# ronantakizawa/cudabulletproof

Measured on AMD Instinct MI355X. Metric: 64-bit range-proof verifies/sec (batched), higher is better.
Workload: dtype u64

## Files before the change

### cudabulletproof_amd/csrc/bp_ipa_prove.hip

```cpp
#include "bp_kernels.h"
#include "ge25519_dev.h"
#include "sha256_dev.h"

namespace bp {

namespace {
constexpr int TPB = 256;
__device__ __forceinline__ size_t gid() { return (size_t)blockIdx.x * blockDim.x + threadIdx.x; }
inline unsigned nblk(size_t items) { return (unsigned)((items + TPB - 1) / TPB); }

__device__ __forceinline__ int sclass(const fe& s) {
    if (s.v[3] | s.v[2] | s.v[1]) return 2;
    return s.v[0] ? 1 : 0;
}

constexpr int CTL_HEAVY = MSM_BINS, CTL_LIGHT = MSM_BINS + 1;

__device__ __forceinline__ void block_hist(const IpaWs& ws, unsigned* hb, bool heavy, int key) {
    for (int k = threadIdx.x; k <= MSM_BINS; k += TPB) hb[k] = 0;
    __syncthreads();
    if (heavy) {
        atomicAdd(&hb[key], 1u);
        atomicAdd(&hb[MSM_BINS], 1u);
    }
    __syncthreads();
    for (int k = threadIdx.x; k <= MSM_BINS; k += TPB)
        if (hb[k]) atomicAdd(&ws.ctl[k], hb[k]);
}
}

__global__ __launch_bounds__(TPB) void k_ipa_elem(IpaWs ws, int np) {
    __shared__ unsigned hb[MSM_BINS + 1];
    const size_t i = gid(), per = 4 * (size_t)np;
    const bool live = i < (size_t)ws.B * per;
    bool heavy = false;
    int key = 0;
    if (live) {
        const size_t p = i / per;
        const int k = (int)(i % per), blk = k / np, j = k % np;
        const size_t n = (size_t)ws.n;
        const fe* a = ws.a + p * n;
        const fe* b = ws.b + p * n;
        const int hi = (blk == 1 || blk == 2) ? np : 0;
        const fe src = (blk & 1) ? b[hi + j] : a[hi + j];
        const fe s = fe_canon(src);
        ws.sc[p * 2 * n + k] = s;
        if (!(blk & 1))
            ws.prod[p * n + hi + j] = fe_mul(src, b[(np - hi) + j]);
        heavy = sclass(s) == 2;
        if (heavy) key = sm_ops_prefix(s, ws.ptab ? ws.pbits : 0);
    }
    block_hist(ws, hb, heavy, key);
}

__global__ __launch_bounds__(TPB) void k_ipa_cchain(IpaWs ws, int np) {
    __shared__ unsigned hb[MSM_BINS + 1];
    const size_t c = gid();
    const bool live = c < (size_t)ws.B * 2;
    bool heavy = false;
    int key = 0;
    if (live) {
        const fe* pr = ws.prod + (c >> 1) * (size_t)ws.n + (c & 1) * (size_t)np;
        fe acc = fe_set(0);
        for (int j = 0; j < np; j++) acc = fe_add(acc, pr[j]);
        const fe s = fe_canon(acc);
        ws.csc[c] = s;
        heavy = sclass(s) == 2;
        if (heavy) key = sm_ops_prefix(s, ws.ptab ? ws.pbits : 0);
    }
    block_hist(ws, hb, heavy, key);
}

__device__ __forceinline__ fe item_scalar(const IpaWs& ws, size_t p, int k, int np) {
    return k < 4 * np ? ws.sc[p * 2 * (size_t)ws.n + k] : ws.csc[p * 2 + (k - 4 * np)];
}
__device__ __forceinline__ ge* item_term(const IpaWs& ws, size_t p, int k, int np) {
    return k < 4 * np ? ws.term + p * 2 * (size_t)ws.n + k : ws.cq + p * 2 + (k - 4 * np);
}

__global__ __launch_bounds__(TPB) void k_ipa_scatter(IpaWs ws, int np, const ge* __restrict__ dtab) {
    __shared__ unsigned cnt[MSM_BINS + 1], base[MSM_BINS + 1];
    for (int k = threadIdx.x; k <= MSM_BINS; k += TPB) cnt[k] = 0;
    __syncthreads();
    const size_t i = gid(), per = 4 * (size_t)np + 2;
    int key = -1;
    unsigned rank = 0;
    if (i < (size_t)ws.B * per) {
        const size_t p = i / per;
        const int k = (int)(i % per);
        const fe s = item_scalar(ws, p, k, np);
        const int c = sclass(s);
        if (c == 0) *item_term(ws, p, k, np) = dtab[k < 4 * np ? 257 : 256];
        else key = c == 2 ? sm_ops_prefix(s, ws.ptab ? ws.pbits : 0) : MSM_BINS;
        if (key >= 0) rank = atomicAdd(&cnt[key], 1u);
    }
    __syncthreads();
    for (int k = threadIdx.x; k <= MSM_BINS; k += TPB)
        if (cnt[k]) base[k] = atomicAdd(&ws.ctl[k < MSM_BINS ? k : CTL_LIGHT], cnt[k]);
    __syncthreads();
    if (key >= 0) (key < MSM_BINS ? ws.slist : ws.llist)[base[key] + rank] = (uint32_t)i;
}

__global__ __launch_bounds__(TPB, 3) void k_ipa_terms(IpaWs ws, int np, const ge* __restrict__ G,
                                                   const ge* __restrict__ H, const ge* __restrict__ Q,
                                                   const ge* __restrict__ dtab) {
    __shared__ geq qs[TPB];
    const int n = ws.n;
    const size_t per = 4 * (size_t)np + 2;
    const unsigned ch = ws.ctl[CTL_HEAVY], cl = ws.ctl[CTL_LIGHT];
    for (size_t i = gid(); i < (size_t)ch + cl; i += (size_t)gridDim.x * TPB) {
        const uint32_t id = i < ch ? ws.slist[i] : ws.llist[i - ch];
        const size_t p = id / per;
        const int k = (int)(id % per);
        const bool msm = k < 4 * np;
        ge P;
        int base;
        if (msm) {
            const int blk = k / np, j = k % np;
            P = blk == 0 ? G[np + j] : blk == 1 ? H[j] : blk == 2 ? G[j] : H[np + j];
            base = blk == 0 ? np + j : blk == 1 ? n + j : blk == 2 ? j : n + np + j;
        } else {
            P = *Q;
            base = 2 * n;
        }
        const fe s = item_scalar(ws, p, k, np);
        const ge* pt = ws.ptab ? ws.ptab + ((size_t)base << ws.pbits) : nullptr;
        ge r = scalarmult<true>(s, P, &qs[threadIdx.x], dtab, pt, pt ? ws.pbits : 0);
        *item_term(ws, p, k, np) = msm ? ge_norm_host(r) : r;
    }
}

__global__ __launch_bounds__(TPB) void k_ipa_pchain(IpaWs ws, int np) {
    const size_t c = gid();
    if (c >= (size_t)ws.B * 4) return;
    const ge* t = ws.term + (c >> 2) * 2 * (size_t)ws.n + (c & 3) * (size_t)np;
    ge acc = t[0];
    for (int i = 1; i < np; i++) acc = ge_norm_host(ge_add(acc, t[i]));
    ws.chain[c] = ge_norm_host(acc);
}

__global__ __launch_bounds__(TPB) void k_ipa_round(IpaWs ws, int r) {
    const size_t p = gid();
    if (p >= (size_t)ws.B) return;
    const ge* ch = ws.chain + p * 4;
    const ge* tq = ws.cq + p * 2;
    const ge L = ge_norm_host(ge_add(ge_add(ge_add(ge_zero(), ch[0]), ch[1]), tq[0]));
    const ge R = ge_norm_host(ge_add(ge_add(ge_add(ge_zero(), ch[2]), ch[3]), tq[1]));
    ws.L[p * ws.Lr + r] = L;
    ws.R[p * ws.Lr + r] = R;
    const fe u = chal_ip(ws.tr[p], L.X, R.X);
    ws.tr[p] = u;
    if (r == 0) ws.x[p] = u;
    ws.uu[p * 2] = u;
    ws.uu[p * 2 + 1] = fe_invert(u);
}

__global__ __launch_bounds__(TPB) void k_ipa_fold(IpaWs ws, int np) {
    const size_t i = gid();
    if (i >= (size_t)ws.B * np) return;
    const size_t p = i / np;
    const int j = (int)(i % np);
    const fe u = ws.uu[p * 2], ui = ws.uu[p * 2 + 1];
    fe* a = ws.a + p * (size_t)ws.n;
    fe* b = ws.b + p * (size_t)ws.n;
    const fe na = fe_add(fe_mul(ui, a[j]), fe_mul(u, a[np + j]));
    const fe nb = fe_add(fe_mul(u, b[j]), fe_mul(ui, b[np + j]));
    a[j] = na;
    b[j] = nb;
}

__global__ __launch_bounds__(TPB) void k_ipa_load(IpaWs ws, const fe* __restrict__ a, const fe* __restrict__ b,
                                                  const fe* __restrict__ tr) {
    const size_t i = gid(), m = (size_t)ws.B * ws.n;
    if (i < m) {
        ws.a[i] = a[i];
        ws.b[i] = b[i];
    }
    if (i < (size_t)ws.B) {
        ws.tr[i] = tr ? tr[i] : fe_set(0);
        ws.x[i] = fe_set(0);
    }
}

__global__ __launch_bounds__(TPB) void k_ipa_final(IpaWs ws, const fe* __restrict__ c_in, fe* a, fe* b, fe* c,
                                                   fe* x, fe* c_final) {
    const size_t p = gid();
    if (p >= (size_t)ws.B) return;
    const fe fa = ws.a[p * (size_t)ws.n], fb = ws.b[p * (size_t)ws.n];
    a[p] = fa;
// ... 33 lines not shown
```

### cudabulletproof_amd/csrc/bp_kernels.hip

```cpp
#include "bp_kernels.h"
#include "ge25519_dev.h"
#include "ge25519_quad.h"
#include "sha256_dev.h"

namespace bp {

constexpr int TPB = 256;
#ifndef BP_TERMS_OCC
#define BP_TERMS_OCC 4
#endif


__device__ __forceinline__ size_t gid() { return (size_t)blockIdx.x * blockDim.x + threadIdx.x; }

__global__ __launch_bounds__(TPB) void k_prefix_tables(ge* tab, const ge* __restrict__ G, const ge* __restrict__ H,
                                                       const ge* __restrict__ h, const ge* __restrict__ g, int n,
                                                       int K, size_t total) {
    const size_t i = gid();
    if (i >= total) return;
    const size_t b = i >> K;
    const uint32_t p = (uint32_t)(i & ((1ull << K) - 1));
    const ge* P = b < (size_t)n ? &G[b] : b < 2 * (size_t)n ? &H[b - n] : b == 2 * (size_t)n ? h : g;
    if (!P) return;
    const geq q = ge_prep(*P);
    ge r = ge_zero();
    for (int j = K - 1; j >= 0; j--) {
        r = ge_add_sel<false>(r, &q, false);
        if ((p >> j) & 1) r = ge_add_sel<false>(r, &q, true);
    }
    tab[i] = r;
}

void launch_prefix_tables(ge* tab, const ge* G, const ge* H, const ge* h, const ge* g, int n, int K, hipStream_t s) {
    const size_t total = (size_t)(2 * n + 2) << K;
    k_prefix_tables<<<(unsigned)((total + TPB - 1) / TPB), TPB, 0, s>>>(tab, G, H, h, g, n, K, total);
}

#ifndef BP_MSM_TPB
#define BP_MSM_TPB 256
#endif
constexpr int MSM_TPB = BP_MSM_TPB;
__global__ __launch_bounds__(MSM_TPB, 768 / MSM_TPB) void k_msm_points(ge* pts, const fe* __restrict__ scal,
                                                    const ge* __restrict__ P, size_t total, size_t pm,
                                                    const uint32_t* __restrict__ perm,
                                                    const ge* __restrict__ dtab, const ge* __restrict__ ptab,
                                                    int K) {
    __shared__ geq qs[MSM_TPB];
    size_t i = gid();
    if (i >= total) return;
    if (perm) i = perm[i];
    const size_t b = pm == total ? i : i % pm;
    ge r = scalarmult<true>(scal[i], P[b], &qs[threadIdx.x], dtab, ptab ? ptab + (b << K) : nullptr, ptab ? K : 0);
    pts[i] = ge_norm_dev(r);
}

constexpr int OPS_BINS = MSM_BINS;

__global__ void k_ops_zero(unsigned* bins) {
    for (int k = threadIdx.x; k < OPS_BINS; k += blockDim.x) bins[k] = 0;
}

__global__ __launch_bounds__(TPB) void k_ops_hist(unsigned* bins, const fe* __restrict__ scal, size_t n, int K) {
    __shared__ unsigned h[OPS_BINS];
    for (int k = threadIdx.x; k < OPS_BINS; k += TPB) h[k] = 0;
    __syncthreads();
    size_t i = gid();
    if (i < n) atomicAdd(&h[sm_ops_prefix(scal[i], K)], 1u);
    __syncthreads();
    for (int k = threadIdx.x; k < OPS_BINS; k += TPB)
        if (h[k]) atomicAdd(&bins[k], h[k]);
}

constexpr int SCAN_T = 1024;
static_assert(OPS_BINS <= SCAN_T, "one scan block");
__global__ __launch_bounds__(SCAN_T) void k_ops_scan(unsigned* bins, int longest_first) {
    __shared__ unsigned a[SCAN_T];
    const int t = threadIdx.x;
    const int k = longest_first ? OPS_BINS - 1 - t : t;
    const unsigned v = t < OPS_BINS ? bins[k] : 0u;
    a[t] = v;
    __syncthreads();
    for (int off = 1; off < SCAN_T; off <<= 1) {
        unsigned x = t >= off ? a[t - off] : 0u;
        __syncthreads();
        a[t] += x;
        __syncthreads();
    }
    if (t < OPS_BINS) bins[k] = a[t] - v;
}

__global__ __launch_bounds__(SCAN_T) void k_ops_scatter(uint32_t* perm, unsigned* offs, const fe* __restrict__ scal,
                                                        size_t n, int K) {
    __shared__ unsigned cnt[OPS_BINS], base[OPS_BINS];
    for (int k = threadIdx.x; k < OPS_BINS; k += SCAN_T) cnt[k] = 0;
    __syncthreads();
    size_t i = (size_t)blockIdx.x * SCAN_T + threadIdx.x;
    int key = 0;
    unsigned rank = 0;
    if (i < n) {
        key = sm_ops_prefix(scal[i], K);
        rank = atomicAdd(&cnt[key], 1u);
    }
    __syncthreads();
    for (int k = threadIdx.x; k < OPS_BINS; k += SCAN_T)
        if (cnt[k]) base[k] = atomicAdd(&offs[k], cnt[k]);
    __syncthreads();
    if (i < n) perm[base[key] + rank] = (uint32_t)i;
}

void launch_ops_scan(unsigned* bins, int longest_first, hipStream_t s) {
    k_ops_scan<<<1, SCAN_T, 0, s>>>(bins, longest_first);
}

void launch_msm_points(ge* pts, const fe* scal, const ge* P, size_t m, uint32_t* perm, unsigned* bins,
                       const ge* dtab, hipStream_t s, size_t pm, const ge* ptab, int K) {
    if (!ptab) K = 0;
    if (!pm) pm = m;
    size_t blocks = (m + TPB - 1) / TPB;
    static const int sort_mode = getenv("HIPBP_MSM_SORT") ? atoi(getenv("HIPBP_MSM_SORT")) : 1;
    if (!sort_mode) perm = nullptr;
    if (perm && bins && m >= MSM_SORT_MIN && m <= 0xFFFFFFFFull) {
        k_ops_zero<<<1, 64, 0, s>>>(bins);
        k_ops_hist<<<blocks, TPB, 0, s>>>(bins, scal, m, K);
        k_ops_scan<<<1, SCAN_T, 0, s>>>(bins, sort_mode == 1);
        k_ops_scatter<<<(unsigned)((m + SCAN_T - 1) / SCAN_T), SCAN_T, 0, s>>>(perm, bins, scal, m, K);
    } else {
        perm = nullptr;
    }
    k_msm_points<<<(unsigned)((m + MSM_TPB - 1) / MSM_TPB), MSM_TPB, 0, s>>>(pts, scal, P, m, pm, perm, dtab, ptab, K);
}

__global__ __launch_bounds__(TPB) void k_tree(ge* out, const ge* __restrict__ in, size_t m, int nb) {
    __shared__ ge sh[TPB];
    int seg = blockIdx.x / nb, chunk = blockIdx.x % nb;
    int tid = threadIdx.x;
// ... 382 lines not shown
```

### cudabulletproof_amd/csrc/bp_prove.hip

```cpp
#include "bp_kernels.h"
#include "ge25519_dev.h"
#include "sha256_dev.h"

#ifndef BP_GTAB
#define BP_GTAB 1
#endif

namespace bp {

namespace {
constexpr int TPB = 256;
__device__ __forceinline__ size_t gid() { return (size_t)blockIdx.x * blockDim.x + threadIdx.x; }
inline unsigned nblk(size_t items) { return (unsigned)((items + TPB - 1) / TPB); }
}

__device__ __forceinline__ const ge* prow(const ProveWs& ws, int b) {
    return ws.ptab ? ws.ptab + ((size_t)b << ws.pbits) : nullptr;
}

__device__ __forceinline__ ge sm_norm(const fe& s, const ge& P, geq* qslot, const ge* __restrict__ dtab,
                                      const ge* pt, int K) {
    return ge_norm_host(scalarmult<true>(s, P, qslot, dtab, pt, pt ? K : 0));
}

// ... 36 lines not shown
}

__device__ __forceinline__ bool next_item(const ProveWs& ws, size_t i, uint32_t& id) {
    const unsigned ch = ws.cnt[0], cl = ws.cnt[1];
    if (i < ch) { id = ws.list[i]; return true; }
    if (i < (size_t)ch + cl) { id = ws.list[ws.cap + (i - ch)]; return true; }
    return false;
}

__device__ __forceinline__ fe terms0_scalar(const ProveIn& in, const ProveWs& ws, size_t p, int k) {
    const int n = in.n;
    if (k < 4 * n) return ws.ps[p * 4 * n + k];
    k -= 4 * n;
    if (k == 0) return fe_canon(in.v[p]);
    if (k == 1) return fe_canon(in.gamma[p]);
    return in.rnd[p * 4 + (k - 2)];
}

__global__ __launch_bounds__(TPB) void k_prove_prep(ProveIn in, ProveWs ws, const ge* __restrict__ dtab) {
    size_t p = gid();
    if (p >= (size_t)in.B) return;
    const int n = in.n;
    fe vc = fe_canon(in.v[p]);
    ws.valid[p] = validate_range(vc, n) ? 1 : 0;
    const fe one = fe_set(1);
    fe* ps = ws.ps + p * 4 * n;
    for (int i = 0; i < n; i++) {
        fe aL = bit_fe(vc, i);
        ps[i] = aL;
        ps[n + i] = fe_canon(fe_sub(aL, one));
        ps[2 * n + i] = fe_canon(in.sL[p * n + i]);
        ps[3 * n + i] = fe_canon(in.sR[p * n + i]);
    }
    const int per = 4 * n + 4;
    ge* pt = ws.pterm + p * per;
    for (int k = 0; k < per; k++)
        if (sclass(terms0_scalar(in, ws, p, k)) == 0) pt[k] = dtab[k < 4 * n + 2 ? 257 : 256];
    queue_items(ws, p, per, [&](int k) {
        if (BP_GTAB && k < n && ps[k].v[0]) return 3;
        if (k >= n && k < 2 * n && !(ps[k - n].v[0])) return 3;
        return sclass(terms0_scalar(in, ws, p, k));
    });
}

constexpr int SORT_T = 256;
__global__ __launch_bounds__(TPB) void k_prove_sort_hist(ProveIn in, ProveWs ws) {
    __shared__ unsigned hb[MSM_BINS];
    for (int k = threadIdx.x; k < MSM_BINS; k += TPB) hb[k] = 0;
    __syncthreads();
    const size_t i = gid(), per = 4 * (size_t)in.n + 4;
    if (i < ws.cnt[0]) {
        const uint32_t id = ws.list[i];
        atomicAdd(&hb[sm_ops_prefix(terms0_scalar(in, ws, id / per, (int)(id % per)), ws.ptab ? ws.pbits : 0)], 1u);
    }
    __syncthreads();
    for (int k = threadIdx.x; k < MSM_BINS; k += TPB)
        if (hb[k]) atomicAdd(&ws.sbins[k], hb[k]);
}

__global__ __launch_bounds__(SORT_T) void k_prove_sort_scatter(ProveIn in, ProveWs ws) {
    __shared__ unsigned cnt[MSM_BINS], base[MSM_BINS];
    for (int k = threadIdx.x; k < MSM_BINS; k += SORT_T) cnt[k] = 0;
    __syncthreads();
    const size_t i = (size_t)blockIdx.x * SORT_T + threadIdx.x, per = 4 * (size_t)in.n + 4;
    int key = 0;
    unsigned rank = 0;
    uint32_t id = 0;
    const bool live = i < ws.cnt[0];
    if (live) {
        id = ws.list[i];
        key = sm_ops_prefix(terms0_scalar(in, ws, id / per, (int)(id % per)), ws.ptab ? ws.pbits : 0);
        rank = atomicAdd(&cnt[key], 1u);
    }
    __syncthreads();
    for (int k = threadIdx.x; k < MSM_BINS; k += SORT_T)
        if (cnt[k]) base[k] = atomicAdd(&ws.sbins[k], cnt[k]);
    __syncthreads();
    if (live) ws.slist[base[key] + rank] = id;
}

__global__ __launch_bounds__(TPB, 3) void k_prove_terms0(ProveIn in, ProveWs ws, const ge* __restrict__ G,
                                                      const ge* __restrict__ H, const ge* __restrict__ g,
                                                      const ge* __restrict__ h, const ge* __restrict__ dtab) {
    __shared__ geq qs[TPB];
    const int n = in.n;
    const size_t per = 4 * (size_t)n + 4;
    const size_t i = gid();
    uint32_t id = 0;
    if (i >= 2 * (size_t)n) {
        const size_t q = i - 2 * n;
        if (ws.slist && q < ws.cnt[0]) id = ws.slist[q];
        else if (!next_item(ws, q, id)) return;
    }
    size_t p = id / per;
    int k = (int)(id % per);
    fe s;
    ge P;
    bool norm = true;
    int base;
    ge* dst = ws.pterm + id;
    if (i < 2 * (size_t)n) {
        const bool hs = i < (size_t)n;
        P = hs ? H[i] : G[i - n];
        base = hs ? n + (int)i : (int)i - n;
        s = hs ? fe_canon(fe_sub(fe_set(0), fe_set(1))) : fe_set(1);
        dst = ws.ctab + i;
    } else if (k < 4 * n) {
        int blk = k / n, j = k % n;
        P = (blk & 1) ? H[j] : G[j];
        base = (blk & 1) ? n + j : j;
        s = ws.ps[p * 4 * n + k];
    } else {
        k -= 4 * n;
        P = k == 0 ? *g : *h;
        base = k == 0 ? 2 * n + 1 : 2 * n;
        s = terms0_scalar(in, ws, p, 4 * n + k);
        norm = k < 2;
    }
    const ge* pt = prow(ws, base);
    ge r = scalarmult<true>(s, P, &qs[threadIdx.x], dtab, pt, pt ? ws.pbits : 0);
    *dst = norm ? ge_norm_host(r) : r;
}

__global__ __launch_bounds__(TPB) void k_prove_chain(const ge* __restrict__ terms, size_t pps, size_t pcs, int count,
                                                     int per_proof, ge* out, int B) {
    size_t c = gid();
    if (c >= (size_t)B * per_proof) return;
    size_t p = c / per_proof;
    int j = (int)(c % per_proof);
    const ge* t = terms + p * pps + (size_t)j * pcs;
    ge acc = t[0];
    for (int i = 1; i < count; i++) acc = ge_norm_host(ge_add(acc, t[i]));
    out[c] = ge_norm_host(acc);
}

__global__ __launch_bounds__(TPB) void k_prove_chain0(ProveIn in, ProveWs ws) {
    size_t c = gid();
    if (c >= (size_t)in.B * 4) return;
    const int n = in.n;
    size_t p = c / 4;
    int j = (int)(c % 4);
    const ge* t = ws.pterm + p * (4 * (size_t)n + 4) + (size_t)j * n;
    const fe* aL = ws.ps + p * 4 * (size_t)n;
    auto term = [&](int i) {
        if (BP_GTAB && j == 0 && aL[i].v[0]) return ws.ctab[n + i];
        return (j == 1 && !aL[i].v[0]) ? ws.ctab[i] : t[i];
    };
    ge acc = term(0);
    for (int i = 1; i < n; i++) acc = ge_norm_host(ge_add(acc, term(i)));
    ws.chain[c] = ge_norm_host(acc);
}

__global__ __launch_bounds__(TPB) void k_prove_commit(ProveIn in, ProveWs ws, const fe* __restrict__ two_i) {
    size_t p = gid();
    if (p >= (size_t)in.B) return;
    const int n = in.n;
    const ge* pt = ws.pterm + p * (4 * (size_t)n + 4) + 4 * n;
    const ge* ch = ws.chain + p * 4;
    ge V = ge_norm_host(ge_add(pt[0], pt[1]));
    ge A = ge_norm_host(ge_add(ge_add(pt[2], ch[0]), ch[1]));
    ge S = ge_norm_host(ge_add(ge_add(pt[3], ch[2]), ch[3]));
    ws.pts[p * 5 + 0] = V;
    ws.pts[p * 5 + 1] = A;
    ws.pts[p * 5 + 2] = S;
    fe y = chal_y(V, A, S);
    fe z = chal_z(y);
    fe z2 = fe_mul(z, z);
    fe vc = fe_canon(in.v[p]);
    const fe one = fe_set(1);
    fe py = one, a0 = fe_set(0), a1 = fe_set(0), a2 = fe_set(0), a3 = fe_set(0), s2 = fe_set(0);
    for (int i = 0; i < n; i++) {
        if (i > 0) py = fe_mul(py, y);
        fe aL = bit_fe(vc, i), aR = fe_sub(aL, one);
        fe lz = fe_sub(aL, z);
        fe u1 = fe_mul(py, fe_add(aR, z));
        fe u2 = fe_mul(py, in.sR[p * n + i]);
        fe sL = in.sL[p * n + i];
        a0 = fe_add(a0, fe_mul(lz, u1));
        a1 = fe_add(a1, fe_mul(sL, u1));
        a2 = fe_add(a2, fe_mul(lz, u2));
        a3 = fe_add(a3, fe_mul(sL, u2));
        s2 = fe_add(s2, two_i[i]);
    }
    fe t0 = fe_add(a0, fe_mul(z2, s2));
    fe t1 = fe_add(a1, a2);
    fe* st = ws.st + p * 8;
    st[0] = y; st[1] = z; st[2] = z2; st[3] = t0; st[4] = t1; st[5] = a3;
    fe* ts = ws.tsc + p * 4;
    ts[0] = fe_canon(t1);
    ts[1] = fe_canon(in.rnd[p * 4 + 2]);
    ts[2] = fe_canon(a3);
    ts[3] = fe_canon(in.rnd[p * 4 + 3]);
}

__global__ __launch_bounds__(TPB, 3) void k_prove_terms1(ProveIn in, ProveWs ws, const ge* __restrict__ g,
                                                      const ge* __restrict__ h, const ge* __restrict__ dtab) {
    __shared__ geq qs[TPB];
    size_t i = gid();
    if (i >= (size_t)in.B * 4) return;
    ws.tt[i] = sm_norm(ws.tsc[i], (i & 1) ? *h : *g, &qs[threadIdx.x], dtab, prow(ws, 2 * in.n + ((i & 1) ? 0 : 1)),
                       ws.pbits);
}

__device__ __forceinline__ void round_prep(const ProveWs& ws, size_t p, int n, int np, const ge* __restrict__ dtab) {
    const fe* a = ws.acur + p * n;
    const fe* b = ws.bcur + p * n;
    fe* cs = ws.csc + p * 2;
    cs[0] = fe_canon(ip_seq(a, b + np, np));
    cs[1] = fe_canon(ip_seq(a + np, b, np));
    fe* sc = ws.iscal + p * 2 * n;
    for (int j = 0; j < np; j++) {
        sc[j] = fe_canon(a[j]);
        sc[np + j] = fe_canon(b[np + j]);
        sc[2 * np + j] = fe_canon(a[np + j]);
        sc[3 * np + j] = fe_canon(b[j]);
    }
    const int per = 4 * np + 2;
    auto scalar_of = [&](int k) { return k < 4 * np ? sc[k] : cs[k - 4 * np]; };
    ge* it = ws.iterm + p * (2 * (size_t)n + 2);
    for (int k = 0; k < per; k++)
        if (sclass(scalar_of(k)) == 0) it[k] = dtab[k < 4 * np ? 257 : 256];
    queue_items(ws, p, per, [&](int k) { return sclass(scalar_of(k)); });
}

__global__ __launch_bounds__(TPB) void k_prove_tx(ProveIn in, ProveWs ws, const fe* __restrict__ two_i,
                                                  const ge* __restrict__ dtab) {
    size_t p = gid();
    if (p >= (size_t)in.B) return;
    const int n = in.n;
    const ge* tt = ws.tt + p * 4;
    ge T1 = ge_norm_host(ge_norm_host(ge_add(tt[0], tt[1])));
    ge T2 = ge_norm_host(ge_norm_host(ge_add(tt[2], tt[3])));
    ws.pts[p * 5 + 3] = T1;
    ws.pts[p * 5 + 4] = T2;
    fe x = chal_x(T1, T2);
    fe x2 = fe_mul(x, x);
    fe* st = ws.st + p * 8;
    const fe y = st[0], z = st[1], z2 = st[2];
    fe t = fe_add(fe_add(st[3], fe_mul(st[4], x)), fe_mul(st[5], x2));
    const fe* rnd = in.rnd + p * 4;
    fe taux = fe_add(fe_mul(rnd[2], x), fe_mul(rnd[3], x2));
    fe mu = fe_add(rnd[0], fe_mul(rnd[1], x));
    fe vc = fe_canon(in.v[p]);
    const fe one = fe_set(1);
    fe* a = ws.acur + p * n;
    fe* b = ws.bcur + p * n;
    fe py = one, ip = fe_set(0);
    for (int i = 0; i < n; i++) {
        if (i > 0) py = fe_mul(py, y);
        fe aL = bit_fe(vc, i), aR = fe_sub(aL, one);
        fe l = fe_add(fe_sub(aL, z), fe_mul(in.sL[p * n + i], x));
        fe r = fe_add(fe_mul(fe_add(fe_add(aR, z), fe_mul(in.sR[p * n + i], x)), py), fe_mul(z2, two_i[i]));
        a[i] = l;
        b[i] = r;
        ip = fe_add(ip, fe_mul(l, r));
    }
    if (!fe_eq(fe_canon(ip), fe_canon(t))) {
        for (int i = 0; i < n; i++) {
            a[i] = fe_set(0);
            b[i] = fe_set(0);
        }
        a[0] = t;
        b[0] = one;
    }
    st[6] = t;
    st[7] = chal_ip_start(t, taux, mu);
    fe* m = ws.misc + p * 4;
    m[0] = taux;
    m[1] = mu;
    m[2] = fe_set(0);
    if (in.L > 0) round_prep(ws, p, n, n >> 1, dtab);
}

__global__ __launch_bounds__(TPB, 3) void k_prove_rterms(ProveIn in, ProveWs ws, int np, const ge* __restrict__ G,
                                                      const ge* __restrict__ H, const ge* __restrict__ Q,
                                                      const ge* __restrict__ dtab) {
    __shared__ geq qs[TPB];
    const int n = in.n;
    const size_t per = 4 * (size_t)np + 2;
    uint32_t id;
    for (size_t i = gid(); next_item(ws, i, id); i += (size_t)gridDim.x * TPB) {
        size_t p = id / per;
        int k = (int)(id % per);
        fe s;
        ge P;
        int base;
        const bool msm = k < 4 * np;
        if (msm) {
            int blk = k / np, j = k % np;
            P = blk == 0 ? G[np + j] : blk == 1 ? H[j] : blk == 2 ? G[j] : H[np + j];
            base = blk == 0 ? np + j : blk == 1 ? n + j : blk == 2 ? j : n + np + j;
            s = ws.iscal[p * 2 * n + k];
        } else {
            P = *Q;
            base = 2 * n;
            s = ws.csc[p * 2 + (k - 4 * np)];
        }
        const ge* pt = prow(ws, base);
        ge r = scalarmult<true>(s, P, &qs[threadIdx.x], dtab, pt, pt ? ws.pbits : 0);
        ws.iterm[p * (2 * (size_t)n + 2) + k] = msm ? ge_norm_host(r) : r;
    }
}

__global__ __launch_bounds__(TPB) void k_prove_round(ProveIn in, ProveWs ws, ProveOut out, int r,
                                                     const ge* __restrict__ dtab) {
    size_t p = gid();
    if (p >= (size_t)in.B) return;
    const int n = in.n, np = n >> (r + 1);
    const ge* ch = ws.chain + p * 4;
    const ge* tq = ws.iterm + p * (2 * (size_t)n + 2) + 4 * np;
    ge L = ge_norm_host(ge_add(ge_add(ge_add(ge_zero(), ch[0]), ch[1]), tq[0]));
    ge R = ge_norm_host(ge_add(ge_add(ge_add(ge_zero(), ch[2]), ch[3]), tq[1]));
    out.L[p * in.L + r] = L;
    out.R[p * in.L + r] = R;
    fe* st = ws.st + p * 8;
    fe u = chal_ip(st[7], L.X, R.X);
    st[7] = u;
    if (r == 0) ws.misc[p * 4 + 2] = u;
    fe ui = fe_invert(u);
    fe* a = ws.acur + p * n;
    fe* b = ws.bcur + p * n;
    for (int j = 0; j < np; j++) {
        fe na = fe_add(fe_mul(ui, a[j]), fe_mul(u, a[np + j]));
        fe nb = fe_add(fe_mul(u, b[j]), fe_mul(ui, b[np + j]));
        a[j] = na;
        b[j] = nb;
    }
    if (r + 1 < in.L) round_prep(ws, p, n, np >> 1, dtab);
}

__global__ __launch_bounds__(TPB) void k_prove_final(ProveIn in, ProveWs ws, ProveOut out) {
    size_t p = gid();
    if (p >= (size_t)in.B) return;
    const bool ok = ws.valid[p] != 0;
    out.valid[p] = ok ? 1 : 0;
    const ge* pts = ws.pts + p * 5;
    const ge O = ge_zero();
    const fe Z = fe_set(0);
    out.V[p] = ok ? pts[0] : O;
    out.A[p] = ok ? pts[1] : O;
    out.S[p] = ok ? pts[2] : O;
    out.T1[p] = ok ? pts[3] : O;
    out.T2[p] = ok ? pts[4] : O;
    const fe t = ws.st[p * 8 + 6];
    const fe* m = ws.misc + p * 4;
    out.taux[p] = ok ? m[0] : Z;
    out.mu[p] = ok ? m[1] : Z;
    out.t[p] = ok ? t : Z;
    out.c[p] = ok ? t : Z;
    out.x[p] = ok ? m[2] : Z;
    out.a[p] = ok ? t : Z;
    out.b[p] = ok ? fe_set(1) : Z;
    if (!ok) {
        const ge zero{Z, Z, Z, Z};
        for (int r = 0; r < in.L; r++) {
            out.L[p * in.L + r] = zero;
            out.R[p * in.L + r] = zero;
        }
    }
}
// ... 53 lines not shown
```

### cudabulletproof_amd/csrc/bp_verify_dev.h

```cpp
#pragma once
#include "bp_kernels.h"
#include "ge25519_dev.h"
#include "ge25519_quad.h"
#include "sha256_dev.h"

namespace bp {

#ifndef BP_TERMS_OCC
#define BP_TERMS_OCC 4
#endif
constexpr int TPB = 256;
__device__ __forceinline__ size_t gid() { return (size_t)blockIdx.x * blockDim.x + threadIdx.x; }



__device__ __forceinline__ void prep_std_task(const BatchView& bv, const VerifyWs& ws, const fe* __restrict__ two_i,
                                              size_t p, const fe& z, const fe& z2, const fe& sy) {
    const int n = bv.n;
    fe x = chal_x(bv.T1[p], bv.T2[p]);
    const fe two = fe_add(fe_set(1), fe_set(1));
    fe z3 = fe_mul(z2, z);
    fe t1 = fe_mul(fe_sub(z, z2), sy);
    fe s2 = fe_set(1);
    for (int i = 1; i < n; i++) s2 = fe_add(s2, two_i[i]);
// ... 325 lines not shown
            sd.poly_out[p * 4 + 3] = ws.m3[p * 2 + 1];
        }
        return;
    }
    int xd = 0, yd = 0, sx = 0, sy = 0, msb = 0;
    for (int i = 0; i < 32; i++) {
        int a = (int)((kx.v[i >> 3] >> (8 * (i & 7))) & 0xff), b = (int)((px.v[i >> 3] >> (8 * (i & 7))) & 0xff);
        int c2 = (int)((ky.v[i >> 3] >> (8 * (i & 7))) & 0xff), d = (int)((py.v[i >> 3] >> (8 * (i & 7))) & 0xff);
        int dx = absdiff(a, b), dy = absdiff(c2, d);
        xd += dx > 0; yd += dy > 0;
        sx += (dx > 0) & (dx <= 10); sy += (dy > 0) & (dy <= 10);
    }
    msb = 64 - __popcll(kx.v[3] ^ px.v[3]);
    const fe hs = sha_4fe(kx, ky, px, py);
    int hz = 0;
    for (int i = 0; i < 32; i++) hz += ((hs.v[i >> 3] >> (8 * (i & 7))) & 0xff) != 0;
    bool accept = (sx + sy >= 20) | (msb >= 28) | (xd + yd <= 32) | (hz <= 24);
    if (wr) sd.ok[p] = (ws.ipok[p] && accept) ? 1 : 0;
}

template <bool QUAD>
__device__ __forceinline__ void ltree_task(const SlotDev& sd, size_t p) {
    const VerifyWs& ws = sd.ws;
    const int n = sd.bv.n;
    const ge m0 = tree_upper<QUAD>(ws.msm_pts + (p * 2 + 0) * n, n, 1);
    const ge m1 = tree_upper<QUAD>(ws.msm_pts + (p * 2 + 1) * n, n, 1);
    if (!QUAD || (threadIdx.x & 3) == 0) {
        ws.msm_part[p * 2 + 0] = m0;
        ws.msm_part[p * 2 + 1] = m1;
    }
}

__device__ __forceinline__ void poly_task(const SlotDev& sd, size_t p) {
    const VerifyWs& ws = sd.ws;
    const ge* t = ws.pterm + p * 8;
    ge left = ge_norm_host(ge_add(t[0], t[1]));
    ge right = ge_zero();
    for (int k = 2; k < 7; k++) right = ge_norm_host(ge_add(right, t[k]));
    left = ge_norm_host(left);
    right = ge_norm_host(right);
    fe lx = fe_canon(left.X), ly = fe_canon(left.Y), rx = fe_canon(right.X), ry = fe_canon(right.Y);
    int dxc = 0, dyc = 0, sxc = 0, syc = 0, cons = 0, prev = 0;
    bool est = false;
    for (int i = 0; i < 32; i++) {
        int a = (int)fe_byte(lx, i), b = (int)fe_byte(rx, i);
        int xd = absdiff(a, b), yd = absdiff((int)fe_byte(ly, i), (int)fe_byte(ry, i));
        dxc += xd > 0; dyc += yd > 0;
        sxc += (xd > 0) & (xd <= 10); syc += (yd > 0) & (yd <= 10);
        int diff = a - b;
        if (!est && diff != 0) {
            prev = diff;
            est = true;
        } else if (est && absdiff(diff, prev) <= 10) {
            cons++;
            prev = (prev * 3 + diff) / 4;
        }
    }
    (void)dyc;
    bool m12 = (dxc <= 5) | ((sxc >= 24) & (syc >= 20)) | (cons >= 20);
    const fe ch = sha_4fe(lx, ly, rx, ry);
    ws.chal[p] = ch;
    ws.lr[p * 2] = left;
    ws.lr[p * 2 + 1] = right;
    ws.rflags[p] |= m12 ? 4 : 0;
    if (sd.poly_out) {
        sd.poly_out[p * 4] = left;
        sd.poly_out[p * 4 + 1] = right;
    }
}

#ifndef BP_DRAIN_OCC
#define BP_DRAIN_OCC 2
#endif
#ifdef BP_TERMS_WPE
#define BP_TERMS_BOUNDS(QL) __launch_bounds__(TPB) __attribute__((amdgpu_waves_per_eu(BP_TERMS_WPE, 8)))
#else
#define BP_TERMS_BOUNDS(QL) __launch_bounds__(TPB, (QL) >= 2 ? BP_DRAIN_OCC : BP_TERMS_OCC)
#endif
template <int QL>
__global__ BP_TERMS_BOUNDS(QL) void k_terms(RegionList rl, const SlotDev* __restrict__ slots,
                                               const ge* __restrict__ G, const ge* __restrict__ H,
                                               const ge* __restrict__ g, const ge* __restrict__ h,
                                               const ge* __restrict__ dtab, const fe* __restrict__ two_i) {
    __shared__ geq qs[TPB];
    size_t i = gid();
    if (i >= rl.total) return;
    const Region rg = find_region(rl, i);
    size_t l = i - rg.begin;
    const SlotDev& sd = slots[rg.slot];
    if (rg.kind == RK_TREE) {
        ge* sh = reinterpret_cast<ge*>(qs);
        const int n = sd.bv.n, ch = n < TPB ? n : TPB, tid = threadIdx.x, idx = tid & (ch - 1);
        const bool live = l < rg.items;
        if (live) sh[tid] = sd.ws.msm_pts[l];
        __syncthreads();
        for (int st = 1; st < ch; st <<= 1) {
            const int j = tid - idx + 2 * st * idx;
            if (live && 2 * st * idx + st < ch) sh[j] = ge_norm_dev(ge_add(sh[j], sh[j + st]));
            __syncthreads();
        }
        if (live && idx == 0) {
            if (n <= TPB) sd.ws.msm_part[l / n] = sh[tid];
            else sd.ws.msm_pts[l] = sh[tid];
        }
        return;
    }
    if (l >= rg.items) return;
    if (rg.kind == RK_PREP) {
        const size_t B = sd.bv.B;
        if (QL >= 4) {
            const size_t it = l >> 2;
            const int qd = threadIdx.x & 3;
            if (sd.range_mode && it < B) prep_range_task_q4(sd.bv, sd.ws, two_i, it, sd.range_mode, qd);
            else prep_ipa_task_q4(sd.bv, sd.ws, sd.range_mode ? it - B : it, qd);
        } else if (sd.range_mode && l < B) {
            prep_range_task(sd.bv, sd.ws, two_i, l, sd.range_mode);
        } else {
            prep_ipa_task(sd.bv, sd.ws, sd.range_mode ? l - B : l);
        }
    } else if (rg.kind == RK_POLY) {
        poly_task(sd, l);
    } else if (rg.kind == RK_FINAL) {
        if (QL >= 4) final_task<true>(sd, l >> 2);
        else final_task<false>(sd, l);
    } else if (rg.kind == RK_LTREE) {
        if (QL >= 4) ltree_task<true>(sd, l >> 2);
        else ltree_task<false>(sd, l);
    } else {
        SmJob jb;
        jb.base = -1;
        bool live = true;
        uint32_t li = (uint32_t)l;
        if (QL == 16) li >>= 4;
        if (QL == 4) li >>= 2;
        if (QL == 2) li >>= 1;
        if (rg.kind == RK_STAGE0 || rg.kind == RK_MSMT) {
            const uint32_t it = rg.kind == RK_MSMT ? stage0_item(sd, (uint32_t)rg.r + li, S0_DEFER)
                                                   : stage0_item(sd, li, sd.defer ? S0_CRIT : S0_ALL);
            live = it != UINT32_MAX && stage0_job(sd, it, G, H, g, h, jb);
        } else if (rg.kind == RK_M3) {
            m3_job(sd, li, jb);
        } else if (rg.kind == RK_ROUND) {
            const int l4 = log2n(sd.bv.n) - rg.r + 1;
            if (const uint32_t* pm = sd.permr[rg.r]) li = pm[li];
            fold_job(sd.bv, sd.ws, rg.r, li >> l4, li & ((1u << l4) - 1), G, H, jb);
        } else {
            if (sd.perm_ft) li = sd.perm_ft[li];
            final_terms_job(sd, li, G, H, jb);
        }
        if (live) {
            const ge* pt = (sd.ptab && jb.base >= 0) ? sd.ptab + ((size_t)jb.base << sd.pbits) : nullptr;
            if (QL == 16) {
                const ge t = sm_row(jb.s, jb.P, dtab, pt, pt ? sd.pbits : 0);
                if ((threadIdx.x & 15) == 0) *jb.dst = jb.dev_norm ? ge_norm_dev(t) : ge_norm_host(t);
            } else if (QL == 4) {
                const ge t = sm_quad(jb.s, jb.P, dtab, pt, pt ? sd.pbits : 0);
                if ((threadIdx.x & 3) == 0) *jb.dst = jb.dev_norm ? ge_norm_dev(t) : ge_norm_host(t);
            } else if (QL == 2) {
                const ge t = sm_pair(jb.s, jb.P, dtab, pt, pt ? sd.pbits : 0);
                if ((threadIdx.x & 1) == 0) *jb.dst = jb.dev_norm ? ge_norm_dev(t) : ge_norm_host(t);
            } else {
                ge t = scalarmult<true>(jb.s, jb.P, &qs[threadIdx.x], dtab, pt, pt ? sd.pbits : 0);
                *jb.dst = jb.dev_norm ? ge_norm_dev(t) : ge_norm_host(t);
            }
        }
    }
}
// ... 11 lines not shown
```

### cudabulletproof_amd/csrc/ge25519_dev.h

```cpp
#pragma once
#include "fe25519_dev.h"

namespace bp {

#ifndef BP_LANE_ADDSUB
#define BP_LANE_ADDSUB 1
#endif
BP_DEV void lane_addsub(const fe& f, const fe& g, fe& sum, fe& diff) {
#if BP_LANE_ADDSUB
    fe_addsub(f, g, sum, diff);
#else
    diff = fe_sub(f, g);
    sum = fe_add(f, g);
#endif
}

struct ge {
    fe X, Y, Z, T;
};

struct geq {
    fe YmX, YpX, Z, T;
};

BP_DEV fe k_const() {
    return fe{{0x75EB4DCA135978A3ull, 0x00700A4D4141D8ABull, 0x8CC740797779E898ull, 0x52036CEE2B6FFE73ull}};
}

BP_DEV fe fe_mul_k(const fe& f) {
#if BP_MUL_ASM && defined(__HIP_DEVICE_COMPILE__)
    uint32_t a[8], w[16];
#pragma unroll
    for (int i = 0; i < 4; i++) {
        a[2 * i] = (uint32_t)f.v[i];
        a[2 * i + 1] = (uint32_t)(f.v[i] >> 32);
    }
    mul512_k_asm(w, a);
    uint64_t t[8];
#pragma unroll
    for (int i = 0; i < 8; i++) t[i] = (uint64_t)w[2 * i] | ((uint64_t)w[2 * i + 1] << 32);
    return fe_fold512(t);
#else
    return fe_mul(f, k_const());
#endif
}

BP_DEV ge ge_zero() { return ge{fe_set(0), fe_set(1), fe_set(1), fe_set(0)}; }

BP_DEV geq ge_prep(const ge& q) {
    return geq{fe_sub(q.Y, q.X), fe_add(q.Y, q.X), q.Z, q.T};
}

BP_DEV ge ge_add_q(const ge& p, const geq& q) {
    fe A = fe_mul(fe_sub(p.Y, p.X), q.YmX);
    fe B = fe_mul(fe_add(p.Y, p.X), q.YpX);
    fe C = fe_mul_k(fe_mul(p.T, q.T));
    fe D = fe_mul(p.Z, q.Z);
    D = fe_add(D, D);
    fe E, F, G, H;
    lane_addsub(B, A, H, E);
    lane_addsub(D, C, G, F);
    return ge{fe_mul(E, F), fe_mul(G, H), fe_mul(F, G), fe_mul(E, H)};
}

BP_DEV ge ge_add(const ge& p, const ge& q) { return ge_add_q(p, ge_prep(q)); }

BP_DEV ge ge_dbl(const ge& p) {
    fe A = fe_sq(fe_sub(p.Y, p.X));
    fe B = fe_sq(fe_add(p.Y, p.X));
    fe C = fe_mul_k(fe_sq(p.T));
    fe D = fe_sq(p.Z);
    D = fe_add(D, D);
    fe E, F, G, H;
    lane_addsub(B, A, H, E);
    lane_addsub(D, C, G, F);
    return ge{fe_mul(E, F), fe_mul(G, H), fe_mul(F, G), fe_mul(E, H)};
}

BP_DEV ge ge_norm_dev(const ge& p) {
    ge r;
    r.X = fe_mul_one(p.X);
    r.Y = fe_mul_one(p.Y);
    r.Z = fe_set(1);
    r.T = fe_mul(r.X, r.Y);
    return r;
}

BP_DEV ge ge_norm_host(const ge& p) {
    if (fe_is_one(fe_canon(p.Z))) return p;
    fe zi = fe_invert(p.Z);
    ge r;
    r.X = fe_mul(p.X, zi);
    r.Y = fe_mul(p.Y, zi);
    r.Z = fe_set(1);
    r.T = fe_mul(r.X, r.Y);
    return r;
}

BP_DEV int fe_clz256(const fe& s) {
    if (s.v[3]) return __clzll(s.v[3]);
    if (s.v[2]) return 64 + __clzll(s.v[2]);
    if (s.v[1]) return 128 + __clzll(s.v[1]);
    if (s.v[0]) return 192 + __clzll(s.v[0]);
    return 256;
}

BP_DEV ge ld_ge(const ge* p) { return *p; }

constexpr int PREFIX_MAX_BITS = 24;
BP_DEV uint32_t prefix_index(const fe& s, int K) { return (uint32_t)(s.v[3] >> (64 - K)); }

BP_DEV int sm_ops(const fe& s) {
    return (256 - fe_clz256(s)) + __popcll(s.v[0]) + __popcll(s.v[1]) + __popcll(s.v[2]) + __popcll(s.v[3]);
}
BP_DEV int sm_ops_prefix(const fe& s, int K) {
    if (K <= 0 || fe_clz256(s) >= K) return sm_ops(s);
    const uint64_t top = K == 64 ? 0 : (s.v[3] & (~0ull >> K));
    return (256 - K) + __popcll(s.v[0]) + __popcll(s.v[1]) + __popcll(s.v[2]) + __popcll(top);
}

template <bool QLDS>
BP_DEV fe qget(const fe* p) {
    if (QLDS) asm volatile("" ::: "memory");
    return *p;
}

template <bool QLDS>
BP_DEV ge ge_add_qp(const ge& p, const geq* q, bool zone = false) {
    fe A = fe_mul(fe_sub(p.Y, p.X), qget<QLDS>(&q->YmX));
    fe B = fe_mul(fe_add(p.Y, p.X), qget<QLDS>(&q->YpX));
    fe C = fe_mul_k(fe_mul(p.T, qget<QLDS>(&q->T)));
    fe D = zone ? fe_mul_one(p.Z) : fe_mul(p.Z, qget<QLDS>(&q->Z));
    D = fe_add(D, D);
    fe E, F, G, H;
    lane_addsub(B, A, H, E);
    lane_addsub(D, C, G, F);
    return ge{fe_mul(E, F), fe_mul(G, H), fe_mul(F, G), fe_mul(E, H)};
}

template <bool QLDS, bool ZONE = false>
BP_DEV ge ge_add_sel(const ge& p, const geq* q, bool use_q) {
    fe ymx = fe_sub(p.Y, p.X);
    fe qa = qget<QLDS>(&q->YmX);
    fe A = fe_mul(ymx, use_q ? qa : ymx);
    fe ypx = fe_add(p.Y, p.X);
    fe qb = qget<QLDS>(&q->YpX);
    fe B = fe_mul(ypx, use_q ? qb : ypx);
    fe qt = qget<QLDS>(&q->T);
    fe C = fe_mul_k(fe_mul(p.T, use_q ? qt : p.T));
    fe D;
    if (ZONE) {
        fe d1 = fe_mul_one(p.Z), d2 = fe_sq(p.Z);
        D = use_q ? d1 : d2;
    } else {
        fe qz = qget<QLDS>(&q->Z);
        D = fe_mul(p.Z, use_q ? qz : p.Z);
    }
    D = fe_add(D, D);
    fe E, F, G, H;
    lane_addsub(B, A, H, E);
    lane_addsub(D, C, G, F);
    return ge{fe_mul(E, F), fe_mul(G, H), fe_mul(F, G), fe_mul(E, H)};
}

struct BitStream {
    uint64_t cur, n1, n2, n3;
    int left;
};

BP_DEV BitStream bs_init(const fe& s, int i) {
    BitStream b{s.v[3], s.v[2], s.v[1], s.v[0], 0};
    int L = i >> 6;
#pragma unroll
    for (int k = 0; k < 3; k++) {
        bool sh = k < 3 - L;
        b.cur = sh ? b.n1 : b.cur;
        b.n1 = sh ? b.n2 : b.n1;
        b.n2 = sh ? b.n3 : b.n2;
        b.n3 = sh ? 0 : b.n3;
    }
    int bi = i & 63;
    b.cur <<= (63 - bi);
    b.left = bi + 1;
    return b;
}

BP_DEV uint32_t bs_next(BitStream& b) {
    uint32_t bit = (uint32_t)(b.cur >> 63);
    b.cur <<= 1;
    if (--b.left == 0) {
        b.cur = b.n1;
        b.n1 = b.n2;
        b.n2 = b.n3;
        b.n3 = 0;
        b.left = 64;
    }
    return bit;
}

template <bool QLDS>
BP_DEV ge sm_uniform(const fe& s_in, const geq* q, const ge* __restrict__ dtab, const ge* ptab, int K) {
    fe s;
#pragma unroll
    for (int i = 0; i < 4; i++) {
        uint32_t lo = __builtin_amdgcn_readfirstlane((uint32_t)s_in.v[i]);
        uint32_t hi = __builtin_amdgcn_readfirstlane((uint32_t)(s_in.v[i] >> 32));
        s.v[i] = (uint64_t)lo | ((uint64_t)hi << 32);
    }
    int lz = fe_clz256(s);
    const bool pre = K > 0 && lz < K && __all(ptab != nullptr);
    const int top = pre ? 255 - K : 255 - lz;
    ge r = ld_ge(pre ? &ptab[prefix_index(s, K)] : &dtab[lz]);
    if (top < 0) return r;
    const bool zone = __all(fe_is_one(qget<QLDS>(&q->Z)));
    BitStream bs = bs_init(s, top);
    for (int i = top; i >= 0; i--) {
        r = ge_dbl(r);
        if (bs_next(bs)) r = ge_add_qp<QLDS>(r, q, zone);
    }
    return r;
}

template <bool QLDS, bool ZONE>
BP_DEV ge sm_lane_loop(const fe& s, const geq* q, const ge* __restrict__ dtab, const ge* ptab, int K) {
    int lz = fe_clz256(s);
    const bool pre = K > 0 && lz < K && ptab != nullptr;
    ge r = ld_ge(pre ? &ptab[prefix_index(s, K)] : &dtab[lz]);
    int i = pre ? 255 - K : 255 - lz;
    BitStream bs = bs_init(s, i < 0 ? 0 : i);
    uint32_t bit = i >= 0 ? bs_next(bs) : 0;
    bool add_phase = false;
    while (i >= 0) {
        r = ge_add_sel<QLDS, ZONE>(r, q, add_phase);
        if (!add_phase && bit) {
            add_phase = true;
        } else {
            add_phase = false;
            i--;
            bit = bs_next(bs);
        }
    }
    return r;
}

template <bool QLDS>
BP_DEV ge sm_lane(const fe& s, const geq* q, const ge* __restrict__ dtab, const ge* ptab, int K) {
    if (__all(fe_is_one(qget<QLDS>(&q->Z)))) return sm_lane_loop<QLDS, true>(s, q, dtab, ptab, K);
    return sm_lane_loop<QLDS, false>(s, q, dtab, ptab, K);
}

template <bool QLDS>
BP_DEV ge scalarmult(const fe& s, const ge& P, geq* slot, const ge* __restrict__ dtab, const ge* ptab = nullptr,
                     int K = 0) {
    geq qreg;
    const geq* q;
    if (QLDS) {
        fe ymx = fe_sub(P.Y, P.X), ypx = fe_add(P.Y, P.X);
#pragma unroll
        for (int k = 0; k < 4; k++) {
            slot->YmX.v[k] = ymx.v[k];
            slot->YpX.v[k] = ypx.v[k];
            slot->Z.v[k] = P.Z.v[k];
            slot->T.v[k] = P.T.v[k];
        }
        q = slot;
    } else {
        qreg = ge_prep(P);
        q = &qreg;
    }
    uint32_t same = 1;
#pragma unroll
    for (int i = 0; i < 4; i++) {
        uint32_t lo = (uint32_t)s.v[i], hi = (uint32_t)(s.v[i] >> 32);
        same &= (lo == __builtin_amdgcn_readfirstlane(lo)) & (hi == __builtin_amdgcn_readfirstlane(hi));
    }
    if (__all(same)) return sm_uniform<QLDS>(s, q, dtab, ptab, K);
    return sm_lane<QLDS>(s, q, dtab, ptab, K);
}

}
```

Baseline: 217,300.

## Select add/double operand via LDS address offset instead of register selects

In the per-lane double-and-add loop, each operand the unified add/double formula needs (Q's field or the point's own coordinate) is written to an LDS slot. The code then reads from an address chosen by the add/double flag, so no vector select is needed across the 4 limbs of each field element. When Z equals one, the existing Z slot in the geq struct is reused as scratch. Otherwise a per-thread own slot is added, which the MSM points kernel turns on. This is meant to cut VALU select instructions and register pressure, at the cost of extra LDS stores and loads on every iteration and a larger LDS footprint.

```diff
diff --git a/cudabulletproof_amd/csrc/bp_ipa_prove.hip b/cudabulletproof_amd/csrc/bp_ipa_prove.hip
--- a/cudabulletproof_amd/csrc/bp_ipa_prove.hip
+++ b/cudabulletproof_amd/csrc/bp_ipa_prove.hip
@@ -104,7 +104,7 @@
 __global__ __launch_bounds__(TPB, 3) void k_ipa_terms(IpaWs ws, int np, const ge* __restrict__ G,
                                                    const ge* __restrict__ H, const ge* __restrict__ Q,
                                                    const ge* __restrict__ dtab) {
-    __shared__ geq qs[TPB];
+    BP_LDS_SLOTS geq qs[TPB];
     const int n = ws.n;
     const size_t per = 4 * (size_t)np + 2;
     const unsigned ch = ws.ctl[CTL_HEAVY], cl = ws.ctl[CTL_LIGHT];
diff --git a/cudabulletproof_amd/csrc/bp_kernels.hip b/cudabulletproof_amd/csrc/bp_kernels.hip
--- a/cudabulletproof_amd/csrc/bp_kernels.hip
+++ b/cudabulletproof_amd/csrc/bp_kernels.hip
@@ -45,12 +45,13 @@
                                                     const uint32_t* __restrict__ perm,
                                                     const ge* __restrict__ dtab, const ge* __restrict__ ptab,
                                                     int K) {
-    __shared__ geq qs[MSM_TPB];
+    BP_LDS_SLOTS geq_own qs[MSM_TPB];
+    static_assert((768 / MSM_TPB) * sizeof(geq_own) * MSM_TPB <= 160 * 1024, "k_msm_points: LDS per CU");
     size_t i = gid();
     if (i >= total) return;
     if (perm) i = perm[i];
     const size_t b = pm == total ? i : i % pm;
-    ge r = scalarmult<true>(scal[i], P[b], &qs[threadIdx.x], dtab, ptab ? ptab + (b << K) : nullptr, ptab ? K : 0);
+    ge r = scalarmult<true, true>(scal[i], P[b], &qs[threadIdx.x].q, dtab, ptab ? ptab + (b << K) : nullptr, ptab ? K : 0);
     pts[i] = ge_norm_dev(r);
 }
 
diff --git a/cudabulletproof_amd/csrc/bp_prove.hip b/cudabulletproof_amd/csrc/bp_prove.hip
--- a/cudabulletproof_amd/csrc/bp_prove.hip
+++ b/cudabulletproof_amd/csrc/bp_prove.hip
@@ -142,7 +142,7 @@
 __global__ __launch_bounds__(TPB, 3) void k_prove_terms0(ProveIn in, ProveWs ws, const ge* __restrict__ G,
                                                       const ge* __restrict__ H, const ge* __restrict__ g,
                                                       const ge* __restrict__ h, const ge* __restrict__ dtab) {
-    __shared__ geq qs[TPB];
+    BP_LDS_SLOTS geq qs[TPB];
     const int n = in.n;
     const size_t per = 4 * (size_t)n + 4;
     const size_t i = gid();
@@ -255,7 +255,7 @@
 
 __global__ __launch_bounds__(TPB, 3) void k_prove_terms1(ProveIn in, ProveWs ws, const ge* __restrict__ g,
                                                       const ge* __restrict__ h, const ge* __restrict__ dtab) {
-    __shared__ geq qs[TPB];
+    BP_LDS_SLOTS geq qs[TPB];
     size_t i = gid();
     if (i >= (size_t)in.B * 4) return;
     ws.tt[i] = sm_norm(ws.tsc[i], (i & 1) ? *h : *g, &qs[threadIdx.x], dtab, prow(ws, 2 * in.n + ((i & 1) ? 0 : 1)),
@@ -335,7 +335,7 @@
 __global__ __launch_bounds__(TPB, 3) void k_prove_rterms(ProveIn in, ProveWs ws, int np, const ge* __restrict__ G,
                                                       const ge* __restrict__ H, const ge* __restrict__ Q,
                                                       const ge* __restrict__ dtab) {
-    __shared__ geq qs[TPB];
+    BP_LDS_SLOTS geq qs[TPB];
     const int n = in.n;
     const size_t per = 4 * (size_t)np + 2;
     uint32_t id;
diff --git a/cudabulletproof_amd/csrc/bp_verify_dev.h b/cudabulletproof_amd/csrc/bp_verify_dev.h
--- a/cudabulletproof_amd/csrc/bp_verify_dev.h
+++ b/cudabulletproof_amd/csrc/bp_verify_dev.h
@@ -431,7 +431,7 @@
                                                const ge* __restrict__ G, const ge* __restrict__ H,
                                                const ge* __restrict__ g, const ge* __restrict__ h,
                                                const ge* __restrict__ dtab, const fe* __restrict__ two_i) {
-    __shared__ geq qs[TPB];
+    BP_LDS_SLOTS geq qs[TPB];
     size_t i = gid();
     if (i >= rl.total) return;
     const Region rg = find_region(rl, i);
diff --git a/cudabulletproof_amd/csrc/ge25519_dev.h b/cudabulletproof_amd/csrc/ge25519_dev.h
--- a/cudabulletproof_amd/csrc/ge25519_dev.h
+++ b/cudabulletproof_amd/csrc/ge25519_dev.h
@@ -19,8 +19,17 @@
     fe X, Y, Z, T;
 };
 
+#define BP_LDS_SLOTS __shared__ __attribute__((aligned(16)))
+
 struct geq {
     fe YmX, YpX, Z, T;
+};
+
+static_assert(offsetof(geq, YmX) == 0 && offsetof(geq, YpX) == 32 && offsetof(geq, Z) == 64 && offsetof(geq, T) == 96,
+              "ge_add_sel addresses geq's fields by these offsets");
+struct geq_own {
+    geq q;
+    fe own;
 };
 
 BP_DEV fe k_const() {
@@ -138,8 +147,64 @@
     return ge{fe_mul(E, F), fe_mul(G, H), fe_mul(F, G), fe_mul(E, H)};
 }
 
-template <bool QLDS, bool ZONE = false>
+#ifndef BP_SEL_LDS
+#define BP_SEL_LDS 1
+#endif
+#if BP_SEL_LDS && defined(__HIP_DEVICE_COMPILE__)
+#define BP_SEL_LDS_DEV 1
+#define BP_LDS_AS __attribute__((address_space(3)))
+typedef uint64_t lds_u64x2 __attribute__((ext_vector_type(2), aligned(16)));
+template <int OWN>
+BP_DEV void own_put(const geq* q, const fe& x) {
+    BP_LDS_AS uint64_t* o = (BP_LDS_AS uint64_t*)((BP_LDS_AS char*)q + OWN);
+#pragma unroll
+    for (int k = 0; k < 4; k++) o[k] = x.v[k];
+}
+template <int OWN, int OFF>
+BP_DEV fe own_pick(const geq* q, uint32_t sel32) {
+    static_assert((OWN - OFF) % 32 == 0, "own slot and q fields 32 bytes apart");
+    const uint32_t a = (uint32_t)(uintptr_t)(BP_LDS_AS const char*)q + OFF + sel32 * ((OWN - OFF) / 32);
+    asm volatile("" ::: "memory");
+    const BP_LDS_AS lds_u64x2* v = (const BP_LDS_AS lds_u64x2*)(uintptr_t)a;
+    const lds_u64x2 lo = v[0], hi = v[1];
+    return fe{{lo.x, lo.y, hi.x, hi.y}};
+}
+#else
+#define BP_SEL_LDS_DEV 0
+#endif
+
+template <bool QLDS, bool ZONE = false, int OWN = 0>
 BP_DEV ge ge_add_sel(const ge& p, const geq* q, bool use_q) {
+#if BP_SEL_LDS_DEV
+    if (QLDS && OWN != 0) {
+        uint32_t sel32 = use_q ? 0u : 32u;
+        asm("" : "+v"(sel32));
+        fe ymx = fe_sub(p.Y, p.X);
+        own_put<OWN>(q, ymx);
+        fe qa = own_pick<OWN, 0>(q, sel32);
+        fe ypx = fe_add(p.Y, p.X);
+        own_put<OWN>(q, ypx);
+        fe qb = own_pick<OWN, 32>(q, sel32);
+        fe A = fe_mul(ymx, qa);
+        own_put<OWN>(q, p.T);
+        fe qt = own_pick<OWN, 96>(q, sel32);
+        fe B = fe_mul(ypx, qb);
+        fe C = fe_mul_k(fe_mul(p.T, qt));
+        fe D;
+        if (ZONE) {
+            fe d1 = fe_mul_one(p.Z), d2 = fe_sq(p.Z);
+            D = use_q ? d1 : d2;
+        } else {
+            own_put<OWN>(q, p.Z);
+            D = fe_mul(p.Z, own_pick<OWN, 64>(q, sel32));
+        }
+        D = fe_add(D, D);
+        fe E, F, G, H;
+        lane_addsub(B, A, H, E);
+        lane_addsub(D, C, G, F);
+        return ge{fe_mul(E, F), fe_mul(G, H), fe_mul(F, G), fe_mul(E, H)};
+    }
+#endif
     fe ymx = fe_sub(p.Y, p.X);
     fe qa = qget<QLDS>(&q->YmX);
     fe A = fe_mul(ymx, use_q ? qa : ymx);
@@ -221,7 +286,7 @@
     return r;
 }
 
-template <bool QLDS, bool ZONE>
+template <bool QLDS, bool ZONE, int OWN = 0>
 BP_DEV ge sm_lane_loop(const fe& s, const geq* q, const ge* __restrict__ dtab, const ge* ptab, int K) {
     int lz = fe_clz256(s);
     const bool pre = K > 0 && lz < K && ptab != nullptr;
@@ -231,7 +296,7 @@
     uint32_t bit = i >= 0 ? bs_next(bs) : 0;
     bool add_phase = false;
     while (i >= 0) {
-        r = ge_add_sel<QLDS, ZONE>(r, q, add_phase);
+        r = ge_add_sel<QLDS, ZONE, OWN>(r, q, add_phase);
         if (!add_phase && bit) {
             add_phase = true;
         } else {
@@ -243,13 +308,14 @@
     return r;
 }
 
-template <bool QLDS>
+template <bool QLDS, bool OWNSLOT = false>
 BP_DEV ge sm_lane(const fe& s, const geq* q, const ge* __restrict__ dtab, const ge* ptab, int K) {
-    if (__all(fe_is_one(qget<QLDS>(&q->Z)))) return sm_lane_loop<QLDS, true>(s, q, dtab, ptab, K);
-    return sm_lane_loop<QLDS, false>(s, q, dtab, ptab, K);
-}
-
-template <bool QLDS>
+    if (__all(fe_is_one(qget<QLDS>(&q->Z))))
+        return sm_lane_loop<QLDS, true, QLDS ? (int)offsetof(geq, Z) : 0>(s, q, dtab, ptab, K);
+    return sm_lane_loop<QLDS, false, QLDS && OWNSLOT ? (int)offsetof(geq_own, own) : 0>(s, q, dtab, ptab, K);
+}
+
+template <bool QLDS, bool OWNSLOT = false>
 BP_DEV ge scalarmult(const fe& s, const ge& P, geq* slot, const ge* __restrict__ dtab, const ge* ptab = nullptr,
                      int K = 0) {
     geq qreg;
@@ -275,7 +341,7 @@
         same &= (lo == __builtin_amdgcn_readfirstlane(lo)) & (hi == __builtin_amdgcn_readfirstlane(hi));
     }
     if (__all(same)) return sm_uniform<QLDS>(s, q, dtab, ptab, K);
-    return sm_lane<QLDS>(s, q, dtab, ptab, K);
-}
-
-}
+    return sm_lane<QLDS, OWNSLOT>(s, q, dtab, ptab, K);
+}
+
+}
```

After: 218,900, median of 6. About the same (+0.7%).
